# sony/timbre-trap

Measured on AMD Instinct MI355X. Metric: audio-seconds/s training throughput (9oct x 60bpo, 3s@22.05kHz), higher is better.
Workload: dtype bf16; 1 GPU; full train step (CQT x2 + AE fwd/bwd with consistency + 3 losses + clip + AdamW), model_complexity=2 latent=128, 64 clips x 3 s per GPU, under torch.autocast like reference experiments/train.py:415 (bf16 MFMA conv path of BASELINE config[2]; fp32 master weights, losses and optimizer); global_batch=64, parallelism=dp1

## Files before the change

timbre-trap_amd/csrc/latent_bf16.hip:

```cpp
#include "bf16_common.h"

namespace {

#ifndef LAT_WGRAD_WAVES
#define LAT_WGRAD_WAVES 4
#endif
#ifndef LAT_EXPAND_Q
#define LAT_EXPAND_Q 2
#endif
#ifndef LAT_NSPLIT
#define LAT_NSPLIT 32
#endif

__device__ __forceinline__ float gate_f(float dy, float y) { return dy * elu_dout(y); }

template <int CT> __device__ __forceinline__ int ochc(int ct, int m) { return (CT / 4) * (m >> 2) + 4 * ct + (m & 3); }

template <int CT, int DT>
__global__ __launch_bounds__(NT) void k_lat_wprep1(const float* __restrict__ w, e16* __restrict__ wp, int D, int E) {
    constexpr int SPH = CT / 32;
    const int i = blockIdx.x * NT + threadIdx.x;
    if (i >= E * SPH * DT * 64) return;
    const int lane = i & 63, dt = (i >> 6) % DT, s = (i >> 6) / DT;
    const int h = s / SPH, half = s - h * SPH;
    const int d = 16 * dt + (lane & 15), c0 = 32 * half + 8 * (lane >> 4);
    e16x8 v;
#pragma unroll
    for (int e = 0; e < 8; ++e) v[e] = (e16)(d < D ? w[((long)d * CT + c0 + e) * E + h] : 0.f);
    reinterpret_cast<e16x8*>(wp)[i] = v;
}
template <int CT, int KS>
__global__ __launch_bounds__(NT) void k_lat_wprep2(const float* __restrict__ w, e16* __restrict__ wp, int D, int E) {
    constexpr int NC = CT / 16;
    const int i = blockIdx.x * NT + threadIdx.x;
    if (i >= E * NC * KS * 64) return;
    const int lane = i & 63, s = (i >> 6) % KS, ct = ((i >> 6) / KS) % NC, h = (i >> 6) / (KS * NC);
    const int c = ochc<CT>(ct, lane & 15), d0 = 32 * s + 8 * (lane >> 4);
    e16x8 v;
#pragma unroll
    for (int e = 0; e < 8; ++e) v[e] = (e16)(d0 + e < D ? w[((long)(d0 + e) * CT + c) * E + h] : 0.f);
    reinterpret_cast<e16x8*>(wp)[i] = v;
}
template <int KS>
__global__ __launch_bounds__(NT) void k_lat_zprep(const float* __restrict__ z, e16* __restrict__ zt, int D, int Dz, float fill, int T,
                                                   long npix, float zscale, int one_row = -1) {
    constexpr int ZS = 32 * KS + 16, PCS = ZS / 8;
    const long i = (long)blockIdx.x * NT + threadIdx.x;
    const long pix = (i / (64 * PCS)) * 64 + (i & 63);
    if (pix >= npix) return;
    const int d0 = (int)((i >> 6) % PCS) * 8;
    const long b = pix / T, t = pix - b * T;
    e16x8 v;
#pragma unroll
    for (int e = 0; e < 8; ++e)
        v[e] = (e16)(zscale * (d0 + e < Dz ? z[(b * Dz + d0 + e) * T + t] : (d0 + e < D ? fill : (d0 + e == one_row ? 1.f : 0.f))));
    *reinterpret_cast<e16x8*>(zt + pix * ZS + d0) = v;
}

template <int CT, int DT, bool GATE, int QN>
__global__ __launch_bounds__(NT) void k_lat_contract(const e16* __restrict__ in, const e16* __restrict__ gy,
                                                      const e16* __restrict__ wp, const float* __restrict__ bias,
                                                      float* __restrict__ out, int D, int Dout, int E, int T, long npix, float oscale) {
    constexpr int SPH = CT / 32;
    constexpr int CHUNK = DT * 64 * 16, ROUNDS = (DT * 64 + NT - 1) / NT;
    extern __shared__ __align__(16) unsigned char smem[];
    const int tid = threadIdx.x, lane = tid & 63, wave = tid >> 6;
    const int n = lane & 15, g = lane >> 4;
    const int nsteps = E * SPH;
    const long p0 = (long)blockIdx.x * (64 * QN) + wave * (16 * QN);
    long pix[QN]; bool ok[QN]; long base[QN];
#pragma unroll
    for (int q = 0; q < QN; ++q) {
        pix[q] = p0 + 16 * q + n;
        ok[q] = pix[q] < npix;
        const long b = pix[q] / T, t = pix[q] - b * T;
        base[q] = (b * E * T + t) * CT + 8 * g;
    }
    auto stage = [&](int s, int buf) {
        const e16* src = wp + (long)s * (DT * 64 * 8);
#pragma unroll
        for (int r = 0; r < ROUNDS; ++r) {
            const int i = r * NT + wave * 64, p = i + lane;
            glds16(src + (long)(p < DT * 64 ? p : DT * 64 - 1) * 8, smem + buf * (ROUNDS * NT * 16) + (long)i * 16);
        }
    };
    auto fetch = [&](int s, e16x8 (&q8)[QN]) {
        const int h = s / SPH, half = s - h * SPH;
#pragma unroll
        for (int q = 0; q < QN; ++q) {
            const long off = base[q] + (long)h * T * CT + 32 * half;
            const bool live = ok[q] && s < nsteps;
            e16x8 v = *reinterpret_cast<const e16x8*>(in + (live ? off : 0));
            if (GATE) {
                const e16x8 yv = *reinterpret_cast<const e16x8*>(gy + (live ? off : 0));
#pragma unroll
                for (int e = 0; e < 8; ++e) v[e] = (e16)gate_f((float)v[e], (float)yv[e]);
            }
            if (!live)
#pragma unroll
                for (int e = 0; e < 8; ++e) v[e] = (e16)0.f;
            q8[q] = v;
        }
    };
    f32x4 acc[DT][QN];
#pragma unroll
    for (int dt = 0; dt < DT; ++dt)
#pragma unroll
        for (int q = 0; q < QN; ++q) acc[dt][q] = f32x4{0.f, 0.f, 0.f, 0.f};
    e16x8 bq[QN], bn[QN];
    stage(0, 0);
    fetch(0, bq);
    for (int s = 0; s < nsteps; ++s) {
        asm volatile("s_waitcnt vmcnt(0)" ::: "memory");
        __syncthreads();
        if (s + 1 < nsteps) stage(s + 1, (s + 1) & 1);
        fetch(s + 1, bn);
        const unsigned char* wb = smem + (s & 1) * (ROUNDS * NT * 16);
#pragma unroll
        for (int dt = 0; dt < DT; ++dt) {
            const e16x8 a = *reinterpret_cast<const e16x8*>(wb + ((long)dt * 64 + lane) * 16);
#pragma unroll
            for (int q = 0; q < QN; ++q) acc[dt][q] = mma32(a, bq[q], acc[dt][q]);
        }
#pragma unroll
        for (int q = 0; q < QN; ++q) bq[q] = bn[q];
    }
#pragma unroll
    for (int q = 0; q < QN; ++q) {
        if (!ok[q]) continue;
        const long b = pix[q] / T, t = pix[q] - b * T;
#pragma unroll
        for (int dt = 0; dt < DT; ++dt)
#pragma unroll
            for (int r = 0; r < 4; ++r) {
                const int d = 16 * dt + 4 * g + r;
                if (d < Dout) out[(b * Dout + d) * T + t] = acc[dt][q][r] * oscale + (bias ? bias[d] : 0.f);
            }
    }
    (void)CHUNK;
}

template <int CT, int KS, bool ACT, int QE, bool GOUT = false>
__global__ __launch_bounds__(NT) void k_lat_expand(const e16* __restrict__ zt, const e16* __restrict__ wp,
                                                    const float* __restrict__ bias, e16* __restrict__ out, int E, int T,
                                                    long npix, const e16* __restrict__ gy = nullptr) {
    constexpr int NC = CT / 16, NCH = CT / 4, ZS = 32 * KS + 16;
    constexpr int PCS = NC * KS * 64, ROUNDS = (PCS + NT - 1) / NT;
    extern __shared__ __align__(16) unsigned char smem[];
    const int tid = threadIdx.x, lane = tid & 63, wave = tid >> 6;
    const int n = lane & 15, g = lane >> 4;
    const long p0 = (long)blockIdx.x * (64 * QE) + wave * (16 * QE);
    e16x8 bz[QE][KS];
    long obase[QE]; bool ok[QE];
#pragma unroll
    for (int q = 0; q < QE; ++q) {
        const long pix = p0 + 16 * q + n;
        ok[q] = pix < npix;
        const long pc = ok[q] ? pix : 0;
#pragma unroll
        for (int s = 0; s < KS; ++s) bz[q][s] = *reinterpret_cast<const e16x8*>(zt + pc * ZS + 32 * s + 8 * g);
        const long b = pc / T, t = pc - b * T;
        obase[q] = (b * E * T + t) * CT + NCH * g;
    }
    float br[NCH];
#pragma unroll
    for (int e = 0; e < NCH; ++e) br[e] = ACT ? bias[NCH * g + e] : 0.f;
    auto stage = [&](int h, int buf) {
        const e16* src = wp + (long)h * (PCS * 8);
#pragma unroll
        for (int r = 0; r < ROUNDS; ++r) {
            const int i = r * NT + wave * 64, p = i + lane;
            glds16(src + (long)(p < PCS ? p : PCS - 1) * 8, smem + buf * (ROUNDS * NT * 16) + (long)i * 16);
        }
    };
    stage(0, 0);
    for (int h = 0; h < E; ++h) {
        asm volatile("s_waitcnt vmcnt(0)" ::: "memory");
        __syncthreads();
        if (h + 1 < E) stage(h + 1, (h + 1) & 1);
        const unsigned char* wb = smem + (h & 1) * (ROUNDS * NT * 16);
        f32x4 acc[NC][QE];
#pragma unroll
        for (int ct = 0; ct < NC; ++ct)
#pragma unroll
            for (int q = 0; q < QE; ++q) acc[ct][q] = f32x4{0.f, 0.f, 0.f, 0.f};
#pragma unroll
        for (int ct = 0; ct < NC; ++ct)
#pragma unroll
            for (int s = 0; s < KS; ++s) {
                const e16x8 a = *reinterpret_cast<const e16x8*>(wb + (((long)ct * KS + s) * 64 + lane) * 16);
#pragma unroll
                for (int q = 0; q < QE; ++q) acc[ct][q] = mma32(a, bz[q][s], acc[ct][q]);
            }
#pragma unroll
        for (int q = 0; q < QE; ++q) {
            if (!ok[q]) continue;
            e16* d = out + obase[q] + (long)h * T * CT;
#pragma unroll
            for (int c8 = 0; c8 < NCH / 8; ++c8) {
                e16x8 o, yv;
                if constexpr (GOUT) yv = *reinterpret_cast<const e16x8*>(gy + obase[q] + (long)h * T * CT + 8 * c8);
#pragma unroll
                for (int e = 0; e < 8; ++e) {
                    const int ch = 8 * c8 + e;
                    const float a = acc[ch >> 2][q][ch & 3] + br[ch];
                    o[e] = (e16)(ACT ? elu_f(a) : (GOUT ? a * elu_dout((float)yv[e]) : a));
                }
                *reinterpret_cast<e16x8*>(d + 8 * c8) = o;
            }
        }
    }
}

template <int CT> __device__ __forceinline__ int gswz(int p) { return CT == 64 ? ((p >> 1) & 3) : ((p >> 2) & 1); }

template <int CT, int DT, int KS, bool GATE>
__global__ __launch_bounds__(NT, LAT_WGRAD_WAVES) void k_lat_wgrad(const e16* __restrict__ zt, const e16* __restrict__ g_in,
                                                   const e16* __restrict__ gy, float* __restrict__ part,
                                                   float* __restrict__ dbpart, int E, int T, long npix, int nsplit) {
    constexpr int NC = CT / 16, ZS = 32 * KS + 16, ZB = ZS * 2, GB = CT * 2;
    constexpr int ZPC = 64 * ZB / 16, GPC = 64 * GB / 16;
    constexpr int ZR = (ZPC + NT - 1) / NT, GR = (GPC + NT - 1) / NT;
    constexpr int WPS = 4 / NC;
    extern __shared__ __align__(16) unsigned char smem[];
    unsigned char* zs = smem;
    unsigned char* gs = smem + ZR * NT * 16;
    const int tid = threadIdx.x, lane = tid & 63, wave = tid >> 6;
    const int n = lane & 15, g = lane >> 4, trj = n >> 2, trq = n & 3;
    const int h = blockIdx.x % E, ps = blockIdx.x / E;
    const int ct = wave % NC, sub0 = wave / NC;
    f32x4 acc[DT];
#pragma unroll
    for (int dt = 0; dt < DT; ++dt) acc[dt] = f32x4{0.f, 0.f, 0.f, 0.f};
    float dbacc[8] = {0.f, 0.f, 0.f, 0.f, 0.f, 0.f, 0.f, 0.f};
    const e16* zero = reinterpret_cast<const e16*>(&g_wzero16);
    const int npx = (int)npix, nchunks = (npx + 63) / 64;
    for (int ck = ps; ck < nchunks; ck += nsplit) {
        const int px0 = ck * 64;
        const int b0 = px0 / T, t00 = px0 - b0 * T;
        __syncthreads();
        const bool full = px0 + 64 <= npx;
        const e16* zc = zt + (long)px0 * ZS;
#pragma unroll
        for (int r = 0; r < ZR; ++r) {
            const int i = r * NT + wave * 64, p = i + lane;
            const bool okp = p < ZPC && (full || px0 + p * 16 / ZB < npx);
            glds16(okp ? zc + p * 8 : zero, zs + (long)i * 16);
        }
        e16x8 v[GATE ? GR : 1], yv[GATE ? GR : 1];
#pragma unroll
        for (int r = 0; r < GR; ++r) {
            const int i = r * NT + wave * 64, p = i + lane;
            const int q = p / (GB / 16), cgp = p % (GB / 16);
            const int cg = (((cgp >> 1) ^ gswz<CT>(q)) << 1) | (cgp & 1);
            const bool okp = p < GPC && (full || px0 + q < npx);
            int b = b0, t = t00 + q;
            if (T >= 64) { if (t >= T) { t -= T; ++b; } }
            else { const int e = t / T; b += e; t -= e * T; }
            const long off = okp ? (long)((b * E + h) * T + t) * CT + cg * 8 : 0;
            if constexpr (!GATE) glds16(okp ? g_in + off : zero, gs + (long)i * 16);
            else { v[r] = *reinterpret_cast<const e16x8*>(g_in + off); yv[r] = *reinterpret_cast<const e16x8*>(gy + off); }
        }
        if constexpr (GATE) {
#pragma unroll
            for (int r = 0; r < GR; ++r) {
                const int p = r * NT + tid;
                const bool okp = p < GPC && px0 + p / (GB / 16) < npx;
                e16x8 o;
#pragma unroll
                for (int e = 0; e < 8; ++e) {
                    const float gq = okp ? gate_f((float)v[r][e], (float)yv[r][e]) : 0.f;
                    dbacc[e] += gq;
                    o[e] = (e16)gq;
                }
                if (p < GPC) *reinterpret_cast<e16x8*>(gs + (long)p * 16) = o;
            }
        }
        asm volatile("s_waitcnt vmcnt(0)" ::: "memory");
        __syncthreads();
        for (int sub = sub0; sub < 2; sub += WPS) {
            s16x4 lo, hi;
            {
                const int p = 32 * sub + 4 * g + trj;
                lo = lds_tr16(gs + (long)p * GB + ((ct ^ gswz<CT>(p)) << 5) + 8 * trq);
                hi = lds_tr16(gs + (long)(p + 16) * GB + ((ct ^ gswz<CT>(p + 16)) << 5) + 8 * trq);
            }
            const e16x8 bq = __builtin_bit_cast(e16x8, __builtin_shufflevector(lo, hi, 0, 1, 2, 3, 4, 5, 6, 7));
#pragma unroll
            for (int dt = 0; dt < DT; ++dt) {
                const int p = 32 * sub + 4 * g + trj;
                const s16x4 alo = lds_tr16(zs + (long)p * ZB + dt * 32 + 8 * trq);
                const s16x4 ahi = lds_tr16(zs + (long)(p + 16) * ZB + dt * 32 + 8 * trq);
                acc[dt] = mma32(__builtin_bit_cast(e16x8, __builtin_shufflevector(alo, ahi, 0, 1, 2, 3, 4, 5, 6, 7)), bq, acc[dt]);
            }
        }
    }
    float* pw = part + ((long)blockIdx.x * 4 + wave) * (DT * 256);
#pragma unroll
    for (int dt = 0; dt < DT; ++dt)
#pragma unroll
        for (int r = 0; r < 4; ++r) pw[(dt * 4 + r) * 64 + lane] = acc[dt][r];
    if constexpr (GATE) {
        __syncthreads();
        float* dl = reinterpret_cast<float*>(smem);
#pragma unroll
        for (int e = 0; e < 8; ++e) dl[tid * 8 + e] = dbacc[e];
        __syncthreads();
        if (tid < CT) {
            float sum = 0.f;
            for (int t2 = 0; t2 < NT; ++t2) {
                const int q = t2 / (GB / 16), cgp = t2 % (GB / 16);
                const int cg = (((cgp >> 1) ^ gswz<CT>(q)) << 1) | (cgp & 1);
                if (cg == (tid >> 3)) sum += dl[t2 * 8 + (tid & 7)];
            }
            dbpart[(long)blockIdx.x * 64 + tid] = sum;
        }
    }
}

template <int CT, int DT>
__global__ __launch_bounds__(NT) void k_lat_wred(const float* __restrict__ part, const float* __restrict__ dbpart, float* __restrict__ dw,
                                                  float* __restrict__ db, int D, int E, int nsplit, float scale, int db_row = -1,
                                                  float* __restrict__ dbrows = nullptr) {
    constexpr int NC = CT / 16, WPS = 4 / NC, WD = DT * 256;
    const int i = blockIdx.x * NT + threadIdx.x;
    const int total = E * NC * WD;
    if (i < total) {
        const int e = i % WD, ct = (i / WD) % NC, h = i / (WD * NC);
        float sum = 0.f;
        for (int ps = 0; ps < nsplit; ++ps)
#pragma unroll
            for (int w2 = 0; w2 < WPS; ++w2) sum += part[(((long)ps * E + h) * 4 + ct + NC * w2) * WD + e];
        const int lane = e & 63, r = (e >> 6) & 3, dt = e >> 8;
        const int d = 16 * dt + 4 * (lane >> 4) + r, c = 16 * ct + (lane & 15);
        if (d < D) dw[((long)d * CT + c) * E + h] += sum * scale;
        else if (d == db_row) dbrows[h * CT + c] = sum * scale;
    } else if (db && db_row < 0 && i < total + CT * 16) {
        const int c = (i - total) % CT, sl = (i - total) / CT;
        float sum = 0.f;
        for (int wg = sl; wg < nsplit * E; wg += 16) sum += dbpart[(long)wg * 64 + c];
        atomicAdd(db + c, sum * scale);
    }
}

__global__ __launch_bounds__(64) void k_lat_dbrows(const float* __restrict__ rows, float* __restrict__ db, int E, int CT) {
    const int c = threadIdx.x;
    if (c >= CT) return;
    float t = 0.f;
    for (int h = 0; h < E; ++h) t += rows[h * CT + c];
    db[c] += t;
}

constexpr int NSPLIT = LAT_NSPLIT;

template <int CT, int DT, int KS> struct LatSizes {
    static constexpr int SPH = CT / 32, NC = CT / 16, ZS = 32 * KS + 16;
    static long wp1_bytes(int E) { return (long)E * SPH * DT * 64 * 16; }
    static long wp2_bytes(int E) { return (long)E * NC * KS * 64 * 16; }
    static long zt_bytes(long npix) { return npix * ZS * 2 + 4096; }
    static long part_bytes(int E) { return ((long)NSPLIT * E * 4 * DT * 256 + (long)NSPLIT * E * 64) * 4; }
};

template <int CT, int DT, int KS, bool GATE>
int run_contract(const e16* in, const e16* gy, const float* w, const float* bias, float* out, unsigned char* ws, int B, int D,
                 int Dout, int E, int T, hipStream_t st, bool pregated = false) {
    using L = LatSizes<CT, DT, KS>;
    const long npix = (long)B * T;
    e16* wp = reinterpret_cast<e16*>(ws);
    const int pieces = E * L::SPH * DT * 64;
    hipLaunchKernelGGL((k_lat_wprep1<CT, DT>), dim3((pieces + NT - 1) / NT), dim3(NT), 0, st, w, wp, D, E);
    TT_LAUNCH_CHECK();
    constexpr int ROUNDS = (DT * 64 + NT - 1) / NT, LDS = 2 * ROUNDS * NT * 16;
    static AttrOnce once;
#ifndef TT_LAT_QN64
#define TT_LAT_QN64 1
#endif
    constexpr int QN = CT == 64 ? TT_LAT_QN64 : 4;
    auto kern = k_lat_contract<CT, DT, GATE, QN>;
    if (int rc = raise_lds(kern, LDS, once)) return rc;
    const float oscale = (GATE || pregated) ? tt_loss_unscale() : 1.f;
    hipLaunchKernelGGL(kern, dim3((unsigned)((npix + 64 * QN - 1) / (64 * QN))), dim3(NT), LDS, st, in, gy, wp, bias, out, D, Dout, E, T, npix, oscale);
    TT_LAUNCH_CHECK();
    return 0;
}

template <int CT, int DT, int KS, bool ACT, bool GOUT = false>
int run_expand(const float* z, int Dz, float fill, const float* w, const float* bias, e16* out, unsigned char* ws, int B, int D, int E,
               int T, hipStream_t st, const e16* gy = nullptr) {
    using L = LatSizes<CT, DT, KS>;
    const long npix = (long)B * T;
    e16* wp = reinterpret_cast<e16*>(ws);
    e16* zt = reinterpret_cast<e16*>(ws + ((L::wp2_bytes(E) + 255) / 256) * 256);
    const int pieces = E * L::NC * KS * 64;
    hipLaunchKernelGGL((k_lat_wprep2<CT, KS>), dim3((pieces + NT - 1) / NT), dim3(NT), 0, st, w, wp, D, E);
    TT_LAUNCH_CHECK();
    const long zp = ((npix + 63) / 64) * 64 * (L::ZS / 8);
    hipLaunchKernelGGL((k_lat_zprep<KS>), dim3((unsigned)((zp + NT - 1) / NT)), dim3(NT), 0, st, z, zt, D, Dz, fill, T, npix,
                       ACT ? 1.f : tt_loss_scale());
    TT_LAUNCH_CHECK();
    constexpr int PCS = L::NC * KS * 64, ROUNDS = (PCS + NT - 1) / NT, LDS = 2 * ROUNDS * NT * 16;
    static AttrOnce once;
    constexpr int QE = LAT_EXPAND_Q;
    auto kern = k_lat_expand<CT, KS, ACT, QE, GOUT>;
    if (int rc = raise_lds(kern, LDS, once)) return rc;
    hipLaunchKernelGGL(kern, dim3((unsigned)((npix + 64 * QE - 1) / (64 * QE))), dim3(NT), LDS, st, zt, wp, bias, out, E, T, npix, gy);
    TT_LAUNCH_CHECK();
    return 0;
}

template <int CT, int DT, int KS, bool GATE>
int run_wgrad(const float* z, int Dz, float fill, const e16* g_in, const e16* gy, float* dw, float* db, unsigned char* ws, int B,
              int D, int E, int T, hipStream_t st, bool pregated = false) {
    using L = LatSizes<CT, DT, KS>;
    const long npix = (long)B * T;
    if (npix >= (1l << 30) || (long)B * E * T >= (1l << 31)) return TT_E_UNSUPPORTED;
    e16* zt = reinterpret_cast<e16*>(ws);
    float* part = reinterpret_cast<float*>(ws + ((L::zt_bytes(npix) + 255) / 256) * 256);
    float* dbpart = part + (long)NSPLIT * E * 4 * DT * 256;
    const long zp = ((npix + 63) / 64) * 64 * (L::ZS / 8);
    if (pregated && (GATE || D >= 16 * DT || !db)) return TT_E_UNSUPPORTED;
    const int one_row = pregated ? D : -1;
    hipLaunchKernelGGL((k_lat_zprep<KS>), dim3((unsigned)((zp + NT - 1) / NT)), dim3(NT), 0, st, z, zt, D, Dz, fill, T, npix,
                       (GATE || pregated) ? 1.f : tt_loss_scale(), one_row);
    TT_LAUNCH_CHECK();
    constexpr int ZB = L::ZS * 2, GBY = CT * 2;
    constexpr int ZR = (64 * ZB / 16 + NT - 1) / NT, GR = (64 * GBY / 16 + NT - 1) / NT;
    constexpr int LDS0 = (ZR + GR) * NT * 16, LDS = LDS0 > NT * 32 ? LDS0 : NT * 32;
    static AttrOnce once;
    auto kern = k_lat_wgrad<CT, DT, KS, GATE>;
    if (int rc = raise_lds(kern, LDS, once)) return rc;
    hipLaunchKernelGGL(kern, dim3(E * NSPLIT), dim3(NT), LDS, st, zt, g_in, gy, part, dbpart, E, T, npix, NSPLIT);
    TT_LAUNCH_CHECK();
    const int total = E * (CT / 16) * DT * 256 + CT * 16;
    hipLaunchKernelGGL((k_lat_wred<CT, DT>), dim3((total + NT - 1) / NT), dim3(NT), 0, st, part, dbpart, dw, (GATE || pregated) ? db : nullptr, D, E,
                       NSPLIT, tt_loss_unscale(), one_row, dbpart);
    TT_LAUNCH_CHECK();
    if (pregated) {
        static_assert(CT <= 64, "one wave sums the channels");
        hipLaunchKernelGGL(k_lat_dbrows, dim3(1), dim3(64), 0, st, dbpart, db, E, CT);
        TT_LAUNCH_CHECK();
    }
    return 0;
}

inline int cfg_of(int CT, int D) {
    if (CT == 32 && D >= 1 && D <= 48) return 1;
    if (CT == 64 && D >= 1 && D <= 144) return 2;
    return 0;
}

}

extern "C" {

int64_t tt_latent16_scratch_bytes(int B, int CT, int D, int E, int T) {
    const long npix = (long)B * T;
    switch (cfg_of(CT, D)) {
        case 1: { using L = LatSizes<32, 3, 2>; return L::wp1_bytes(E) + L::wp2_bytes(E) + L::zt_bytes(npix) + L::part_bytes(E) + 4096; }
        case 2: { using L = LatSizes<64, 9, 5>; return L::wp1_bytes(E) + L::wp2_bytes(E) + L::zt_bytes(npix) + L::part_bytes(E) + 4096; }
    }
    return -1;
}

int tt_latent16_contract(const void* in, const void* gy, const float* w, const float* bias, float* out, void* ws, int B, int CT, int D,
                         int Dout, int E, int T, void* stream) {
    if (!in || !w || !out || !ws || B <= 0 || E <= 0 || T <= 0 || T % 16 || Dout < 1 || Dout > D) return TT_E_BADARG;
    hipStream_t st = tt_stream(stream);
    const e16 *i = (const e16*)in, *y = (const e16*)gy;
    unsigned char* s = (unsigned char*)ws;
    switch (cfg_of(CT, D)) {
        case 1: return y ? run_contract<32, 3, 2, true>(i, y, w, bias, out, s, B, D, Dout, E, T, st) : run_contract<32, 3, 2, false>(i, y, w, bias, out, s, B, D, Dout, E, T, st);
        case 2: return y ? run_contract<64, 9, 5, true>(i, y, w, bias, out, s, B, D, Dout, E, T, st) : run_contract<64, 9, 5, false>(i, y, w, bias, out, s, B, D, Dout, E, T, st);
    }
    return TT_E_UNSUPPORTED;
}

int tt_latent16_expand(const float* z, int Dz, float fill, const float* w, const float* bias, void* out, void* ws, int B, int CT, int D,
                       int E, int T, void* stream) {
    if (!z || !w || !out || !ws || B <= 0 || E <= 0 || T <= 0 || T % 16 || (Dz != D && Dz != D - 1)) return TT_E_BADARG;
    hipStream_t st = tt_stream(stream);
    e16* o = (e16*)out;
    unsigned char* s = (unsigned char*)ws;
    switch (cfg_of(CT, D)) {
        case 1: return bias ? run_expand<32, 3, 2, true>(z, Dz, fill, w, bias, o, s, B, D, E, T, st) : run_expand<32, 3, 2, false>(z, Dz, fill, w, bias, o, s, B, D, E, T, st);
        case 2: return bias ? run_expand<64, 9, 5, true>(z, Dz, fill, w, bias, o, s, B, D, E, T, st) : run_expand<64, 9, 5, false>(z, Dz, fill, w, bias, o, s, B, D, E, T, st);
    }
    return TT_E_UNSUPPORTED;
}

int tt_latent16_wgrad(const float* z, int Dz, float fill, const void* g, const void* gy, float* dw, float* db, void* ws, int B, int CT,
                      int D, int E, int T, void* stream) {
    if (!z || !g || !dw || !ws || (gy && !db) || B <= 0 || E <= 0 || T <= 0 || T % 16 || (Dz != D && Dz != D - 1)) return TT_E_BADARG;
    hipStream_t st = tt_stream(stream);
    const e16 *gi = (const e16*)g, *y = (const e16*)gy;
    unsigned char* s = (unsigned char*)ws;
    switch (cfg_of(CT, D)) {
        case 1: return y ? run_wgrad<32, 3, 2, true>(z, Dz, fill, gi, y, dw, db, s, B, D, E, T, st) : run_wgrad<32, 3, 2, false>(z, Dz, fill, gi, y, dw, db, s, B, D, E, T, st);
        case 2: return y ? run_wgrad<64, 9, 5, true>(z, Dz, fill, gi, y, dw, db, s, B, D, E, T, st) : run_wgrad<64, 9, 5, false>(z, Dz, fill, gi, y, dw, db, s, B, D, E, T, st);
    }
    return TT_E_UNSUPPORTED;
}

int tt_latent16_pregated_ok(int CT, int D) {
    switch (cfg_of(CT, D)) {
        case 1: return D < 16 * 3;
        case 2: return D < 16 * 9;
    }
    return 0;
}

int tt_latent16_expand_gated(const float* z, const float* w, const void* gy, void* out, void* ws, int B, int CT, int D, int E, int T,
                             void* stream) {
    if (!z || !w || !gy || !out || !ws || B <= 0 || E <= 0 || T <= 0 || T % 16) return TT_E_BADARG;
    hipStream_t st = tt_stream(stream);
    switch (cfg_of(CT, D)) {
        case 1: return run_expand<32, 3, 2, false, true>(z, D, 0.f, w, nullptr, (e16*)out, (unsigned char*)ws, B, D, E, T, st, (const e16*)gy);
        case 2: return run_expand<64, 9, 5, false, true>(z, D, 0.f, w, nullptr, (e16*)out, (unsigned char*)ws, B, D, E, T, st, (const e16*)gy);
    }
    return TT_E_UNSUPPORTED;
}

int tt_latent16_contract_pregated(const void* g, const float* w, float* out, void* ws, int B, int CT, int D, int Dout, int E, int T,
                                  void* stream) {
    if (!g || !w || !out || !ws || B <= 0 || E <= 0 || T <= 0 || T % 16 || Dout < 1 || Dout > D) return TT_E_BADARG;
    hipStream_t st = tt_stream(stream);
    switch (cfg_of(CT, D)) {
        case 1: return run_contract<32, 3, 2, false>((const e16*)g, nullptr, w, nullptr, out, (unsigned char*)ws, B, D, Dout, E, T, st, true);
        case 2: return run_contract<64, 9, 5, false>((const e16*)g, nullptr, w, nullptr, out, (unsigned char*)ws, B, D, Dout, E, T, st, true);
    }
    return TT_E_UNSUPPORTED;
}

int tt_latent16_wgrad_pregated(const float* z, int Dz, float fill, const void* g, float* dw, float* db, void* ws, int B, int CT, int D,
                               int E, int T, void* stream) {
    if (!z || !g || !dw || !db || !ws || B <= 0 || E <= 0 || T <= 0 || T % 16 || (Dz != D && Dz != D - 1)) return TT_E_BADARG;
    hipStream_t st = tt_stream(stream);
    switch (cfg_of(CT, D)) {
        case 1: return run_wgrad<32, 3, 2, false>(z, Dz, fill, (const e16*)g, nullptr, dw, db, (unsigned char*)ws, B, D, E, T, st, true);
        case 2: return run_wgrad<64, 9, 5, false>(z, Dz, fill, (const e16*)g, nullptr, dw, db, (unsigned char*)ws, B, D, E, T, st, true);
    }
    return TT_E_UNSUPPORTED;
}

}
```

timbre-trap_amd/csrc/wide_common.h:

```cpp
#pragma once
#include "bf16_common.h"

namespace {

template <int C> __device__ __forceinline__ int chan_of(int ct, int m) { return C == 32 ? 8 * (m >> 2) + 4 * ct + (m & 3) : m; }

template <int C> __device__ __forceinline__ int fswz(int col) {
    return C == 32 ? ((((col >> 2) & 1) << 1) | ((col >> 3) & 1)) : ((col >> 3) & 1);
}

template <int C> struct WK {
    static constexpr int NCT = C / 16;
    static constexpr int NK = C == 32 ? 9 : 5;
    static constexpr int NCH = C == 32 ? 8 : 4;
    static constexpr int W3 = NK * NCT * 64;
    static constexpr int ENTRIES = 2 * W3 + 2 * NCT * 64;
    static constexpr int IMG_BYTES = ENTRIES * 16;
};

template <int C, int D, int IW>
__device__ __forceinline__ void conv_taps(const unsigned char* img, int row, int col, int g,
                                          const e16x8 (&A)[WK<C>::NK][WK<C>::NCT], f32x4 (&acc)[WK<C>::NCT], e16x8& centre) {
    constexpr int NK = WK<C>::NK, NCT = WK<C>::NCT, PB = C * 2;
    const int gsel = C == 32 ? g : (g & 1);
#pragma unroll
    for (int k = 0; k < NK; ++k) {
        int tap = C == 32 ? k : 2 * k + (g >> 1);
        if (tap > 8) tap = 8;
        const int kh = tap / 3, kw = tap - 3 * kh;
        const int xc = col + kw * D;
        const e16x8 bq = *reinterpret_cast<const e16x8*>(img + ((row + kh * D) * IW + xc) * PB + 16 * (gsel ^ fswz<C>(xc)));
        if (C == 32 && k == 4) centre = bq;
#pragma unroll
        for (int ct = 0; ct < NCT; ++ct) acc[ct] = mma32(A[k][ct], bq, acc[ct]);
    }
}

template <class V> __device__ __forceinline__ void gload_ahead(V& dst, const void* base, unsigned off) {
    static_assert(sizeof(V) == 8 || sizeof(V) == 16, "a lane's channels of one pixel");
    if constexpr (sizeof(V) == 8) asm volatile("global_load_dwordx2 %0, %1, %2" : "=v"(dst) : "v"(off), "s"(base) : "memory");
    else asm volatile("global_load_dwordx4 %0, %1, %2" : "=v"(dst) : "v"(off), "s"(base) : "memory");
}
template <class V> __device__ __forceinline__ void gstore_counted(const V& v, void* base, unsigned off) {
    static_assert(sizeof(V) == 8 || sizeof(V) == 16, "a lane's channels of one pixel");
    if constexpr (sizeof(V) == 8) asm volatile("global_store_dwordx2 %0, %1, %2" ::"v"(off), "v"(v), "s"(base) : "memory");
    else asm volatile("global_store_dwordx4 %0, %1, %2\n\ts_nop 1" ::"v"(off), "v"(v), "s"(base) : "memory");
}
template <int N> __device__ __forceinline__ void gload_wait() { asm volatile("s_waitcnt vmcnt(%0)" ::"n"(N) : "memory"); }
template <class V> __device__ __forceinline__ void gload_use(V& v) { asm volatile("" : "+v"(v)); }
template <class V> __device__ __forceinline__ void vmem_retired(const V& v) { asm volatile("" ::"v"(v)); }

constexpr int MAX_A_WG = 2048, MAX_W_WG = 1024;

struct RedArgs {
    const float* pw; int gw;
    const float* pa; int ga;
    float *dw1, *db1, *dw2, *db2;
    int split_a = 0;
    int one_dump = 0;
    float scale = tt_loss_unscale();
};
struct RedBatch { RedArgs a[4]; int n = 0; };
template <int C>
__global__ __launch_bounds__(1024) void k_wrb_reduce(RedBatch batch) {
    const RedArgs& ar = batch.a[blockIdx.y];
    constexpr int NCT = C / 16;
    constexpr int WDUMP = 9 * NCT * 256, NEW = NCT * WDUMP;
    constexpr int ADUMP = C * C + 2 * C;
    __shared__ float red[RSL][REL];
    const int el = threadIdx.x % REL, sl = threadIdx.x / REL;
    const int e = blockIdx.x * REL + el;
    float sum = 0.f;
    float* dst = nullptr;
    if (e < NEW) {
        const int role = e / WDUMP, rest = e - role * WDUMP;
        const int k = rest / (NCT * 256), a = (rest >> 8) % NCT, r = (rest >> 6) & 3, lane = rest & 63;
        const int NS = (ar.split_a || ar.one_dump) ? 1 : 4 / NCT;
        const int ncontrib = ar.gw * NS;
        float part[8] = {0.f, 0.f, 0.f, 0.f, 0.f, 0.f, 0.f, 0.f};
        for (int j0 = sl; j0 < ncontrib; j0 += 8 * RSL) {
#pragma unroll
            for (int u = 0; u < 8; ++u) {
                const int j = j0 + RSL * u;
                if (j < ncontrib) {
                    const int wg = j / NS, s = j - wg * NS;
                    const int wave = ar.split_a ? role + 2 * a : (ar.one_dump ? 0 : (C == 32 ? role + 2 * s : s));
                    part[u] += ar.pw[((long)wg * 4 + wave) * WDUMP + rest];
                }
            }
        }
        sum = ((part[0] + part[1]) + (part[2] + part[3])) + ((part[4] + part[5]) + (part[6] + part[7]));
        const int co = 16 * a + 4 * (lane >> 4) + r, ci = 16 * role + (lane & 15);
        dst = ar.dw1 + (co * C + ci) * 9 + k;
    } else if (e < NEW + ADUMP) {
        const int q = e - NEW;
        const int ncontrib = ar.ga;
        float part[8] = {0.f, 0.f, 0.f, 0.f, 0.f, 0.f, 0.f, 0.f};
        for (int j0 = sl; j0 < ncontrib; j0 += 8 * RSL) {
#pragma unroll
            for (int u = 0; u < 8; ++u) {
                const int j = j0 + RSL * u;
                if (j < ncontrib) part[u] += ar.pa[(long)j * ADUMP + q];
            }
        }
        sum = ((part[0] + part[1]) + (part[2] + part[3])) + ((part[4] + part[5]) + (part[6] + part[7]));
        if (q < C * C) {
            const int a = q / (NCT * 256), c = (q >> 8) % NCT, r = (q >> 6) & 3, lane = q & 63;
            dst = ar.dw2 + (16 * a + 4 * (lane >> 4) + r) * C + 16 * c + (lane & 15);
        } else if (q < C * C + C) dst = ar.db1 + (q - C * C);
        else dst = ar.db2 + (q - C * C - C);
    }
    red[sl][el] = sum;
    __syncthreads();
    if (sl == 0 && dst) {
        float s = 0.f;
#pragma unroll
        for (int i = 0; i < RSL; ++i) s += red[i][el];
        *dst += s * ar.scale;
    }
}

}
struct SkipJ {
    const e16* g = nullptr;
    long half = 0;
    const float* w = nullptr;
    float* dw = nullptr;
    float unscale = 1.f;
};
struct LevelCtx {
    void* red = nullptr;
    bool wprep_done = false;
    bool gate = false;
    SkipJ skip;
    bool gated = false;
};
int ttx_wide_wprep_batch(int C, int n, const float* const* w1, const float* const* w2, void* const* ws, hipStream_t st);
int ttx_wide_rb_bwd_onepass(LevelCtx* ctx, const void* x, const void* h1, const void* dy, const float* w1, const float* w2, const float* b2,
                            void* dx, float* dw1, float* db1, float* dw2, float* db2, void* ws, int B, int C, int H, int T, int dilation,
                            void* stream);
int ttx_wide_bwds_attr(int C, int dilation, int form, int* local_bytes, int* num_regs);
namespace {
template <class Kernel> inline int kernel_attr(Kernel kern, int* local_bytes, int* num_regs) {
    hipFuncAttributes fa;
    hipError_t e = hipFuncGetAttributes(&fa, reinterpret_cast<const void*>(kern));
    if (e != hipSuccess) return (int)e;
    *local_bytes = (int)fa.localSizeBytes;
    *num_regs = fa.numRegs;
    return 0;
}
template <class V, int N>
__device__ __forceinline__ void skipj_terms(const V& g0, const V& g1, bool two, const V& xq, float w, float (&add)[N], float& dot) {
#pragma unroll
    for (int j = 0; j < N; ++j) {
        const float t = two ? (float)g0[j] + (float)g1[j] : (float)g0[j];
        dot = __builtin_fmaf(t, (float)xq[j], dot);
        add[j] = w * t;
    }
}
__device__ __forceinline__ void skipj_finish(float dot, const SkipJ& sj) {
    if (!sj.dw) return;
#pragma unroll
    for (int o = 32; o > 0; o >>= 1) dot += __shfl_xor(dot, o, 64);
    if ((threadIdx.x & 63) == 0) atomicAdd(sj.dw, dot * sj.unscale);
}

enum class FirstForm { Plain, Gated, Riding };
inline FirstForm first_form(LevelCtx* ctx, int D) {
    if (!ctx || !ctx->gate || D != 1) return FirstForm::Plain;
    ctx->gated = true;
    return ctx->skip.g ? FirstForm::Riding : FirstForm::Gated;
}

template <class Kernel> inline int reduce_or_defer(LevelCtx* ctx, Kernel kern, int total, const RedArgs& ra, hipStream_t st, int per_block = REL) {
    if (ctx && ctx->red) {
        RedBatch* b = static_cast<RedBatch*>(ctx->red);
        if (b->n >= 4) return TT_E_BADARG;
        b->a[b->n++] = ra;
        return 0;
    }
    RedBatch one;
    one.a[0] = ra; one.n = 1;
    hipLaunchKernelGGL(kern, dim3((total + per_block - 1) / per_block, 1), dim3(1024), 0, st, one);
    TT_LAUNCH_CHECK();
    return 0;
}

}
```

Measured before the change: 3938 audio-seconds/s.

## Deepen latent contract/expand pipelines with counted vmcnt waits and triple-buffered weights

Rewrites the latent contract kernel to prefetch operands several steps ahead into a register ring and triple-buffer weight stages in LDS. Replaces full vmcnt(0) drains with counted waits and an lgkm-only barrier, and issues LDS reads via inline asm with immediate offsets. The expand kernel overlaps its gated-output loads and stores the same way, QN for CT=64 goes from 1 to 2, and offsets become 32-bit relative to a per-wave base. The aim is to hide global-load latency behind MFMA work, at the cost of more registers and LDS, a new 4GiB offset guard, and a relaxed T%8 check.

```diff
diff --git a/timbre-trap_amd/csrc/latent_bf16.hip b/timbre-trap_amd/csrc/latent_bf16.hip
--- a/timbre-trap_amd/csrc/latent_bf16.hip
+++ b/timbre-trap_amd/csrc/latent_bf16.hip
@@ -1,6 +1,12 @@
-#include "bf16_common.h"
+#include "wide_common.h"
 
 namespace {
+
+constexpr int LAT_OPS_AHEAD = 3, LAT_RING = 3;
+
+template <int I, int N, class F> __device__ __forceinline__ void static_for(F&& f) {
+    if constexpr (I < N) { f(std::integral_constant<int, I>{}); static_for<I + 1, N>(f); }
+}
 
 #ifndef LAT_WGRAD_WAVES
 #define LAT_WGRAD_WAVES 4
@@ -62,44 +68,42 @@
                                                       const e16* __restrict__ wp, const float* __restrict__ bias,
                                                       float* __restrict__ out, int D, int Dout, int E, int T, long npix, float oscale) {
     constexpr int SPH = CT / 32;
-    constexpr int CHUNK = DT * 64 * 16, ROUNDS = (DT * 64 + NT - 1) / NT;
+    constexpr int ROUNDS = (DT * 64 + NT - 1) / NT, BUF = ROUNDS * NT * 16;
+    constexpr int NF = QN * (GATE ? 2 : 1), PER = NF + ROUNDS;
+    constexpr int NSLOT = LAT_OPS_AHEAD + 1;
     extern __shared__ __align__(16) unsigned char smem[];
-    const int tid = threadIdx.x, lane = tid & 63, wave = tid >> 6;
+    const int tid = threadIdx.x, lane = tid & 63, wave = __builtin_amdgcn_readfirstlane(tid >> 6);
     const int n = lane & 15, g = lane >> 4;
     const int nsteps = E * SPH;
     const long p0 = (long)blockIdx.x * (64 * QN) + wave * (16 * QN);
-    long pix[QN]; bool ok[QN]; long base[QN];
+    const long bw = (p0 < npix ? p0 : npix - 1) / T;
+    long pix[QN]; bool ok[QN]; unsigned loff[QN];
 #pragma unroll
     for (int q = 0; q < QN; ++q) {
         pix[q] = p0 + 16 * q + n;
         ok[q] = pix[q] < npix;
         const long b = pix[q] / T, t = pix[q] - b * T;
-        base[q] = (b * E * T + t) * CT + 8 * g;
-    }
+        loff[q] = ok[q] ? (unsigned)((((b - bw) * E * T + t) * CT + 8 * g) * 2) : 0u;
+    }
+    const e16* inw = in + bw * E * T * CT;
+    const e16* gyw = GATE ? gy + bw * E * T * CT : nullptr;
     auto stage = [&](int s, int buf) {
-        const e16* src = wp + (long)s * (DT * 64 * 8);
+        const e16* src = wp + (long)(s < nsteps ? s : nsteps - 1) * (DT * 64 * 8);
 #pragma unroll
         for (int r = 0; r < ROUNDS; ++r) {
             const int i = r * NT + wave * 64, p = i + lane;
-            glds16(src + (long)(p < DT * 64 ? p : DT * 64 - 1) * 8, smem + buf * (ROUNDS * NT * 16) + (long)i * 16);
+            glds16(src + (long)(p < DT * 64 ? p : DT * 64 - 1) * 8, smem + buf * BUF + (long)i * 16);
         }
     };
-    auto fetch = [&](int s, e16x8 (&q8)[QN]) {
-        const int h = s / SPH, half = s - h * SPH;
+    e16x8 bq[NSLOT][QN], by[GATE ? NSLOT : 1][QN];
+    auto fetch = [&](int s, int slot) {
+        const int sc = s < nsteps ? s : nsteps - 1;
+        const int h = sc / SPH, half = sc - h * SPH;
+        const long row = (long)h * T * CT + 32 * half;
 #pragma unroll
         for (int q = 0; q < QN; ++q) {
-            const long off = base[q] + (long)h * T * CT + 32 * half;
-            const bool live = ok[q] && s < nsteps;
-            e16x8 v = *reinterpret_cast<const e16x8*>(in + (live ? off : 0));
-            if (GATE) {
-                const e16x8 yv = *reinterpret_cast<const e16x8*>(gy + (live ? off : 0));
-#pragma unroll
-                for (int e = 0; e < 8; ++e) v[e] = (e16)gate_f((float)v[e], (float)yv[e]);
-            }
-            if (!live)
-#pragma unroll
-                for (int e = 0; e < 8; ++e) v[e] = (e16)0.f;
-            q8[q] = v;
+            gload_ahead(bq[slot][q], inw + row, loff[q]);
+            if constexpr (GATE) gload_ahead(by[slot][q], gyw + row, loff[q]);
         }
     };
     f32x4 acc[DT][QN];
@@ -107,37 +111,85 @@
     for (int dt = 0; dt < DT; ++dt)
 #pragma unroll
         for (int q = 0; q < QN; ++q) acc[dt][q] = f32x4{0.f, 0.f, 0.f, 0.f};
-    e16x8 bq[QN], bn[QN];
-    stage(0, 0);
-    fetch(0, bq);
-    for (int s = 0; s < nsteps; ++s) {
-        asm volatile("s_waitcnt vmcnt(0)" ::: "memory");
-        __syncthreads();
-        if (s + 1 < nsteps) stage(s + 1, (s + 1) & 1);
-        fetch(s + 1, bn);
-        const unsigned char* wb = smem + (s & 1) * (ROUNDS * NT * 16);
-#pragma unroll
-        for (int dt = 0; dt < DT; ++dt) {
-            const e16x8 a = *reinterpret_cast<const e16x8*>(wb + ((long)dt * 64 + lane) * 16);
-#pragma unroll
-            for (int q = 0; q < QN; ++q) acc[dt][q] = mma32(a, bq[q], acc[dt][q]);
-        }
-#pragma unroll
-        for (int q = 0; q < QN; ++q) bq[q] = bn[q];
-    }
+    static_assert(LAT_OPS_AHEAD >= 2 && LAT_RING == 3, "operands at least as far ahead as the weights; two weight stages ahead");
+    static_for<0, LAT_OPS_AHEAD>([&](auto kc) {
+        constexpr int k = decltype(kc)::value;
+        fetch(k, k);
+        if constexpr (k >= LAT_OPS_AHEAD - 2) stage(k - (LAT_OPS_AHEAD - 2), k - (LAT_OPS_AHEAD - 2));
+    });
+    int rb = 0;
+    for (int s0 = 0; s0 < nsteps; s0 += NSLOT) {
+#pragma unroll
+        for (int j = 0; j < NSLOT; ++j) {
+            const int s = s0 + j;
+            if (s >= nsteps) break;
+            gload_wait<PER>();
+            barrier_keep_vmem();
+            fetch(s + LAT_OPS_AHEAD, (j + LAT_OPS_AHEAD) % NSLOT);
+            stage(s + 2, rb == 0 ? 2 : rb - 1);
+            e16x8 b[QN];
+#pragma unroll
+            for (int q = 0; q < QN; ++q) {
+                gload_use(bq[j][q]);
+                e16x8 v = bq[j][q];
+                if constexpr (GATE) {
+                    gload_use(by[j][q]);
+#pragma unroll
+                    for (int e = 0; e < 8; ++e) v[e] = (e16)gate_f((float)v[e], (float)by[j][q][e]);
+                }
+                if (!ok[q])
+#pragma unroll
+                    for (int e = 0; e < 8; ++e) v[e] = (e16)0.f;
+                b[q] = v;
+            }
+            const unsigned wa = lds_addr(smem + rb * BUF) + lane * 16;
+            e16x8 a[DT];
+            static_for<0, DT>([&](auto dt) { lds_read16_asm<dt.value * 1024>(a[dt.value], wa); });
+            lds_wait<0>();
+#pragma unroll
+            for (int dt = 0; dt < DT; ++dt) {
+                gload_use(a[dt]);
+#pragma unroll
+                for (int q = 0; q < QN; ++q) acc[dt][q] = mma32(a[dt], b[q], acc[dt][q]);
+            }
+            rb = rb == 2 ? 0 : rb + 1;
+        }
+    }
+    gload_wait<0>();
+    static_assert(DT % 3 == 0, "row tiles leave in threes");
+    const float* bsrc = bias ? bias : reinterpret_cast<const float*>(&g_wzero16);
+    const int blast = bias ? Dout - 1 : 0;
+    float* orow[QN];
 #pragma unroll
     for (int q = 0; q < QN; ++q) {
-        if (!ok[q]) continue;
-        const long b = pix[q] / T, t = pix[q] - b * T;
-#pragma unroll
-        for (int dt = 0; dt < DT; ++dt)
+        const long pc = ok[q] ? pix[q] : 0, b = pc / T, t = pc - b * T;
+        orow[q] = out + b * Dout * T + t;
+    }
+#pragma unroll
+    for (int d3 = 0; d3 < DT; d3 += 3) {
+        float bv[3][4];
+#pragma unroll
+        for (int dt = 0; dt < 3; ++dt)
 #pragma unroll
             for (int r = 0; r < 4; ++r) {
-                const int d = 16 * dt + 4 * g + r;
-                if (d < Dout) out[(b * Dout + d) * T + t] = acc[dt][q][r] * oscale + (bias ? bias[d] : 0.f);
-            }
-    }
-    (void)CHUNK;
+                const int d = 16 * (d3 + dt) + 4 * g + r;
+                bv[dt][r] = bsrc[d < blast ? d : blast];
+            }
+#pragma unroll
+        for (int dt = 0; dt < 3; ++dt)
+#pragma unroll
+            for (int r = 0; r < 4; ++r) vmem_retired(bv[dt][r]);
+#pragma unroll
+        for (int q = 0; q < QN; ++q) {
+#pragma unroll
+            for (int dt = 0; dt < 3; ++dt)
+#pragma unroll
+                for (int r = 0; r < 4; ++r) {
+                    const int d = 16 * (d3 + dt) + 4 * g + r;
+                    if (ok[q] && d < Dout) orow[q][(long)d * T] = acc[d3 + dt][q][r] * oscale + bv[dt][r];
+                }
+        }
+    }
 }
 
 template <int CT, int KS, bool ACT, int QE, bool GOUT = false>
@@ -146,12 +198,15 @@
                                                     long npix, const e16* __restrict__ gy = nullptr) {
     constexpr int NC = CT / 16, NCH = CT / 4, ZS = 32 * KS + 16;
     constexpr int PCS = NC * KS * 64, ROUNDS = (PCS + NT - 1) / NT;
+    constexpr int BUF = ROUNDS * NT * 16, NST = QE * (NCH / 8);
     extern __shared__ __align__(16) unsigned char smem[];
-    const int tid = threadIdx.x, lane = tid & 63, wave = tid >> 6;
+    const int tid = threadIdx.x, lane = tid & 63, wave = __builtin_amdgcn_readfirstlane(tid >> 6);
     const int n = lane & 15, g = lane >> 4;
     const long p0 = (long)blockIdx.x * (64 * QE) + wave * (16 * QE);
+    const long bw = (p0 < npix ? p0 : npix - 1) / T;
+    const bool full = p0 + 16 * QE <= npix;
     e16x8 bz[QE][KS];
-    long obase[QE]; bool ok[QE];
+    unsigned ooff[QE]; bool ok[QE];
 #pragma unroll
     for (int q = 0; q < QE; ++q) {
         const long pix = p0 + 16 * q + n;
@@ -160,8 +215,10 @@
 #pragma unroll
         for (int s = 0; s < KS; ++s) bz[q][s] = *reinterpret_cast<const e16x8*>(zt + pc * ZS + 32 * s + 8 * g);
         const long b = pc / T, t = pc - b * T;
-        obase[q] = (b * E * T + t) * CT + NCH * g;
-    }
+        ooff[q] = ok[q] ? (unsigned)((((b - bw) * E * T + t) * CT + NCH * g) * 2) : 0u;
+    }
+    e16* outw = out + bw * E * T * CT;
+    const e16* gyw = GOUT ? gy + bw * E * T * CT : nullptr;
     float br[NCH];
 #pragma unroll
     for (int e = 0; e < NCH; ++e) br[e] = ACT ? bias[NCH * g + e] : 0.f;
@@ -170,46 +227,70 @@
 #pragma unroll
         for (int r = 0; r < ROUNDS; ++r) {
             const int i = r * NT + wave * 64, p = i + lane;
-            glds16(src + (long)(p < PCS ? p : PCS - 1) * 8, smem + buf * (ROUNDS * NT * 16) + (long)i * 16);
+            glds16(src + (long)(p < PCS ? p : PCS - 1) * 8, smem + buf * BUF + (long)i * 16);
         }
     };
     stage(0, 0);
+#pragma unroll
+    for (int q = 0; q < QE; ++q)
+#pragma unroll
+        for (int s = 0; s < KS; ++s) vmem_retired(bz[q][s]);
+#pragma unroll
+    for (int e = 0; e < NCH; ++e) vmem_retired(br[e]);
     for (int h = 0; h < E; ++h) {
-        asm volatile("s_waitcnt vmcnt(0)" ::: "memory");
-        __syncthreads();
-        if (h + 1 < E) stage(h + 1, (h + 1) & 1);
-        const unsigned char* wb = smem + (h & 1) * (ROUNDS * NT * 16);
+        if (h == 0 || !full) gload_wait<0>(); else gload_wait<NST>();
+        barrier_keep_vmem();
+        const long row = (long)h * T * CT;
+        e16x8 yv[GOUT ? QE : 1][NCH / 8];
+        if constexpr (GOUT) {
+#pragma unroll
+            for (int q = 0; q < QE; ++q)
+#pragma unroll
+                for (int c8 = 0; c8 < NCH / 8; ++c8) gload_ahead(yv[q][c8], gyw + row + 8 * c8, ooff[q]);
+        }
+        stage(h + 1 < E ? h + 1 : h, (h + 1) & 1);
+        const unsigned wa = lds_addr(smem + (h & 1) * BUF) + lane * 16;
         f32x4 acc[NC][QE];
 #pragma unroll
         for (int ct = 0; ct < NC; ++ct)
 #pragma unroll
             for (int q = 0; q < QE; ++q) acc[ct][q] = f32x4{0.f, 0.f, 0.f, 0.f};
-#pragma unroll
-        for (int ct = 0; ct < NC; ++ct)
+        static_for<0, NC>([&](auto ctc) {
+            constexpr int ct = decltype(ctc)::value;
+            e16x8 a[KS];
+            static_for<0, KS>([&](auto sc) { lds_read16_asm<(ct * KS + decltype(sc)::value) * 1024>(a[decltype(sc)::value], wa); });
+            lds_wait<0>();
 #pragma unroll
             for (int s = 0; s < KS; ++s) {
-                const e16x8 a = *reinterpret_cast<const e16x8*>(wb + (((long)ct * KS + s) * 64 + lane) * 16);
-#pragma unroll
-                for (int q = 0; q < QE; ++q) acc[ct][q] = mma32(a, bz[q][s], acc[ct][q]);
-            }
+                gload_use(a[s]);
+#pragma unroll
+                for (int q = 0; q < QE; ++q) acc[ct][q] = mma32(a[s], bz[q][s], acc[ct][q]);
+            }
+        });
+        if constexpr (GOUT) {
+            gload_wait<ROUNDS>();
+#pragma unroll
+            for (int q = 0; q < QE; ++q)
+#pragma unroll
+                for (int c8 = 0; c8 < NCH / 8; ++c8) gload_use(yv[q][c8]);
+        }
 #pragma unroll
         for (int q = 0; q < QE; ++q) {
             if (!ok[q]) continue;
-            e16* d = out + obase[q] + (long)h * T * CT;
 #pragma unroll
             for (int c8 = 0; c8 < NCH / 8; ++c8) {
-                e16x8 o, yv;
-                if constexpr (GOUT) yv = *reinterpret_cast<const e16x8*>(gy + obase[q] + (long)h * T * CT + 8 * c8);
+                e16x8 o;
 #pragma unroll
                 for (int e = 0; e < 8; ++e) {
                     const int ch = 8 * c8 + e;
                     const float a = acc[ch >> 2][q][ch & 3] + br[ch];
-                    o[e] = (e16)(ACT ? elu_f(a) : (GOUT ? a * elu_dout((float)yv[e]) : a));
+                    o[e] = (e16)(ACT ? elu_f(a) : (GOUT ? a * elu_dout((float)yv[GOUT ? q : 0][c8][e]) : a));
                 }
-                *reinterpret_cast<e16x8*>(d + 8 * c8) = o;
-            }
-        }
-    }
+                gstore_counted(o, outw + row + 8 * c8, ooff[q]);
+            }
+        }
+    }
+    gload_wait<0>();
 }
 
 template <int CT> __device__ __forceinline__ int gswz(int p) { return CT == 64 ? ((p >> 1) & 3) : ((p >> 2) & 1); }
@@ -370,12 +451,13 @@
     const int pieces = E * L::SPH * DT * 64;
     hipLaunchKernelGGL((k_lat_wprep1<CT, DT>), dim3((pieces + NT - 1) / NT), dim3(NT), 0, st, w, wp, D, E);
     TT_LAUNCH_CHECK();
-    constexpr int ROUNDS = (DT * 64 + NT - 1) / NT, LDS = 2 * ROUNDS * NT * 16;
+    constexpr int ROUNDS = (DT * 64 + NT - 1) / NT, LDS = LAT_RING * ROUNDS * NT * 16;
     static AttrOnce once;
 #ifndef TT_LAT_QN64
-#define TT_LAT_QN64 1
+#define TT_LAT_QN64 2
 #endif
     constexpr int QN = CT == 64 ? TT_LAT_QN64 : 4;
+    if (((long)(16 * QN) / T + 2) * E * T * CT * 2 >= (1l << 32)) return TT_E_UNSUPPORTED;
     auto kern = k_lat_contract<CT, DT, GATE, QN>;
     if (int rc = raise_lds(kern, LDS, once)) return rc;
     const float oscale = (GATE || pregated) ? tt_loss_unscale() : 1.f;
@@ -401,6 +483,7 @@
     constexpr int PCS = L::NC * KS * 64, ROUNDS = (PCS + NT - 1) / NT, LDS = 2 * ROUNDS * NT * 16;
     static AttrOnce once;
     constexpr int QE = LAT_EXPAND_Q;
+    if (((long)(16 * QE) / T + 2) * E * T * CT * 2 >= (1l << 32)) return TT_E_UNSUPPORTED;
     auto kern = k_lat_expand<CT, KS, ACT, QE, GOUT>;
     if (int rc = raise_lds(kern, LDS, once)) return rc;
     hipLaunchKernelGGL(kern, dim3((unsigned)((npix + 64 * QE - 1) / (64 * QE))), dim3(NT), LDS, st, zt, wp, bias, out, E, T, npix, gy);
@@ -464,7 +547,7 @@
 
 int tt_latent16_contract(const void* in, const void* gy, const float* w, const float* bias, float* out, void* ws, int B, int CT, int D,
                          int Dout, int E, int T, void* stream) {
-    if (!in || !w || !out || !ws || B <= 0 || E <= 0 || T <= 0 || T % 16 || Dout < 1 || Dout > D) return TT_E_BADARG;
+    if (!in || !w || !out || !ws || B <= 0 || E <= 0 || T <= 0 || T % 8 || Dout < 1 || Dout > D) return TT_E_BADARG;
     hipStream_t st = tt_stream(stream);
     const e16 *i = (const e16*)in, *y = (const e16*)gy;
     unsigned char* s = (unsigned char*)ws;
@@ -477,7 +560,7 @@
 
 int tt_latent16_expand(const float* z, int Dz, float fill, const float* w, const float* bias, void* out, void* ws, int B, int CT, int D,
                        int E, int T, void* stream) {
-    if (!z || !w || !out || !ws || B <= 0 || E <= 0 || T <= 0 || T % 16 || (Dz != D && Dz != D - 1)) return TT_E_BADARG;
+    if (!z || !w || !out || !ws || B <= 0 || E <= 0 || T <= 0 || T % 8 || (Dz != D && Dz != D - 1)) return TT_E_BADARG;
     hipStream_t st = tt_stream(stream);
     e16* o = (e16*)out;
     unsigned char* s = (unsigned char*)ws;
@@ -490,7 +573,7 @@
 
 int tt_latent16_wgrad(const float* z, int Dz, float fill, const void* g, const void* gy, float* dw, float* db, void* ws, int B, int CT,
                       int D, int E, int T, void* stream) {
-    if (!z || !g || !dw || !ws || (gy && !db) || B <= 0 || E <= 0 || T <= 0 || T % 16 || (Dz != D && Dz != D - 1)) return TT_E_BADARG;
+    if (!z || !g || !dw || !ws || (gy && !db) || B <= 0 || E <= 0 || T <= 0 || T % 8 || (Dz != D && Dz != D - 1)) return TT_E_BADARG;
     hipStream_t st = tt_stream(stream);
     const e16 *gi = (const e16*)g, *y = (const e16*)gy;
     unsigned char* s = (unsigned char*)ws;
@@ -511,7 +594,7 @@
 
 int tt_latent16_expand_gated(const float* z, const float* w, const void* gy, void* out, void* ws, int B, int CT, int D, int E, int T,
                              void* stream) {
-    if (!z || !w || !gy || !out || !ws || B <= 0 || E <= 0 || T <= 0 || T % 16) return TT_E_BADARG;
+    if (!z || !w || !gy || !out || !ws || B <= 0 || E <= 0 || T <= 0 || T % 8) return TT_E_BADARG;
     hipStream_t st = tt_stream(stream);
     switch (cfg_of(CT, D)) {
         case 1: return run_expand<32, 3, 2, false, true>(z, D, 0.f, w, nullptr, (e16*)out, (unsigned char*)ws, B, D, E, T, st, (const e16*)gy);
@@ -522,7 +605,7 @@
 
 int tt_latent16_contract_pregated(const void* g, const float* w, float* out, void* ws, int B, int CT, int D, int Dout, int E, int T,
                                   void* stream) {
-    if (!g || !w || !out || !ws || B <= 0 || E <= 0 || T <= 0 || T % 16 || Dout < 1 || Dout > D) return TT_E_BADARG;
+    if (!g || !w || !out || !ws || B <= 0 || E <= 0 || T <= 0 || T % 8 || Dout < 1 || Dout > D) return TT_E_BADARG;
     hipStream_t st = tt_stream(stream);
     switch (cfg_of(CT, D)) {
         case 1: return run_contract<32, 3, 2, false>((const e16*)g, nullptr, w, nullptr, out, (unsigned char*)ws, B, D, Dout, E, T, st, true);
@@ -533,7 +616,7 @@
 
 int tt_latent16_wgrad_pregated(const float* z, int Dz, float fill, const void* g, float* dw, float* db, void* ws, int B, int CT, int D,
                                int E, int T, void* stream) {
-    if (!z || !g || !dw || !db || !ws || B <= 0 || E <= 0 || T <= 0 || T % 16 || (Dz != D && Dz != D - 1)) return TT_E_BADARG;
+    if (!z || !g || !dw || !db || !ws || B <= 0 || E <= 0 || T <= 0 || T % 8 || (Dz != D && Dz != D - 1)) return TT_E_BADARG;
     hipStream_t st = tt_stream(stream);
     switch (cfg_of(CT, D)) {
         case 1: return run_wgrad<32, 3, 2, false>(z, Dz, fill, (const e16*)g, nullptr, dw, db, (unsigned char*)ws, B, D, E, T, st, true);
diff --git a/timbre-trap_amd/csrc/wide_common.h b/timbre-trap_amd/csrc/wide_common.h
--- a/timbre-trap_amd/csrc/wide_common.h
+++ b/timbre-trap_amd/csrc/wide_common.h
@@ -48,6 +48,12 @@
 }
 template <int N> __device__ __forceinline__ void gload_wait() { asm volatile("s_waitcnt vmcnt(%0)" ::"n"(N) : "memory"); }
 template <class V> __device__ __forceinline__ void gload_use(V& v) { asm volatile("" : "+v"(v)); }
+template <int OFF, class V> __device__ __forceinline__ void lds_read16_asm(V& dst, unsigned addr) {
+    static_assert(sizeof(V) == 16 && OFF >= 0 && OFF < 65536, "one ds_read_b128 with an immediate offset");
+    asm volatile("ds_read_b128 %0, %1 offset:%2" : "=v"(dst) : "v"(addr), "n"(OFF) : "memory");
+}
+template <int N> __device__ __forceinline__ void lds_wait() { asm volatile("s_waitcnt lgkmcnt(%0)" ::"n"(N) : "memory"); }
+__device__ __forceinline__ void barrier_keep_vmem() { asm volatile("s_waitcnt lgkmcnt(0)\n\ts_barrier" ::: "memory"); }
 template <class V> __device__ __forceinline__ void vmem_retired(const V& v) { asm volatile("" ::"v"(v)); }
 
 constexpr int MAX_A_WG = 2048, MAX_W_WG = 1024;
```

New measurement: 3937 audio-seconds/s. No clear change (-0.0%).
